# huster-wgm/SRCGAN

Hardware: AMD Instinct MI355X
Metric: paired SR-CycleGAN train images/sec at x4 256->1024 (higher is better)
Workload: dtype bf16; 1 GPU; Sat2Aerx4 paired G+D step (BASELINE configs[1]): 23-block RRDB generator + 3-layer PatchGAN, 3x256x256->3x1024x1024, batch 16/GPU; per_gpu_batch=16, global_batch=16, parallelism=dp1, gradient_exchange=none (1 rank)

## Files before the change

include/srcgan_amd.h:

```cpp
#ifndef SRCGAN_AMD_H
#define SRCGAN_AMD_H

#include <stddef.h>
#include <stdint.h>

#ifdef __cplusplus
extern "C" {
#endif

#define SRCGAN_F32 0
#define SRCGAN_BF16 1
#define SRCGAN_F16 2

int srcgan_version(void);
const char* srcgan_last_error(void);
int srcgan_dtype_size(int dtype);

int srcgan_nchw_f32_to_nhwc(const float* src, void* dst, int B, int C, int H, int W,
                            int cs, int dtype, void* stream);
int srcgan_nhwc_to_nchw_f32(const void* src, float* dst, int B, int C, int H, int W,
                            int cs, int coff, int dtype, void* stream);

size_t srcgan_packed_weight_bytes(int rows, int kdim, int ntaps, int dtype);
int srcgan_pack_weight(const float* w, void* wp, int rows, int kdim, int tys, int txs,
// ... 39 lines not shown
size_t srcgan_conv_wgrad_slab_bytes(int Cout, int Cin, int kh, int kw, int nsplit);
int srcgan_conv_wgrad_nsplit(int B, int OH, int OW, int Cout, int Cin, int stride);
int srcgan_conv_wgrad(const srcgan_wgrad_desc* d, void* stream);

typedef struct srcgan_wgrad_seg { int g0, g1; float* grad; float* bias; int Cin; float alpha; } srcgan_wgrad_seg;
typedef struct srcgan_wgrad_dense_desc {
    const void* dy; const void* x; float* slab;
    int dtype;
    int B, H, W;
    int G, dy_cs, dy_coff;
    int C, x_cs, x_coff;
    int nseg;
    srcgan_wgrad_seg seg[8];
    int accumulate;
    long dy_plane, x_plane;
} srcgan_wgrad_dense_desc;
size_t srcgan_wgrad_dense_slab_bytes(int G, int C, int dtype, int B, int H, int W);
int srcgan_wgrad_dense(const srcgan_wgrad_dense_desc* d, void* stream);

int srcgan_col_reduce_blocks(long npix);
int srcgan_col_reduce(int mode, const void* a, int a_cs, int a_coff, const void* z, int z_cs, int z_coff,
                      const float* m, const float* rstd, long npix, int C, float scale,
                      float* out0, float* out1, float* scratch, int dtype, void* stream);

int srcgan_bn_finalize(const float* mean, const float* var, float* rstd, float* running_mean,
                       float* running_var, int64_t* num_batches_tracked, int C, long count,
                       float momentum, float eps, void* stream);
int srcgan_bn_eval_rstd(const float* running_var, float* rstd, int C, float eps, void* stream);
int srcgan_bn_apply_lrelu(const void* z, void* y, const float* mean, const float* rstd, const float* gamma,
                          const float* beta, long npix, int C, int cs, float slope, int dtype, void* stream);
int srcgan_bn_bwd_apply(const void* g, const void* z, void* dz, const float* mean, const float* rstd,
                        const float* gamma, const float* sum_g, const float* sum_gx, long npix, int C, int cs,
                        int dtype, void* stream);

int srcgan_add_inplace(void* y, int y_cs, int y_coff, const void* x, int x_cs, int x_coff,
                       const void* mz, int mz_cs, int mz_coff, float mslope, long npix, int C, int dtype, void* stream);
int srcgan_add_inplace_planes(void* y, int y_cs, int y_coff, long y_plane, const void* x, int x_cs, int x_coff, long x_plane,
                              const void* mz, int mz_cs, int mz_coff, long mz_plane, float mslope, long npix, int C,
                              int dtype, void* stream);

size_t srcgan_gn_scratch_floats(int B, int C);
int srcgan_gn_forward(const void* x, int x_cs, const void* res, int res_cs, void* y, int y_cs, const float* gamma, const float* beta,
                      float* stats, int B, long hw, int C, int G, float eps, int relu, float slope, int dtype, float* scratch, void* stream);
int srcgan_gn_backward(const void* dy, int dy_cs, const void* yact, int ya_cs, const void* x, int x_cs, const float* gamma, const float* stats,
                       void* dx, int dx_cs, void* dres, int dres_cs, int dres_accumulate, float* dgamma, float* dbeta, int accumulate,
                       float slope, int B, long hw, int C, int G, int dtype, float* scratch, void* stream);

size_t srcgan_ca_scratch_floats(int B, long hw, int C);
int srcgan_ca_forward(const void* t, int t_cs, const void* res, int res_cs, void* y, int y_cs, const float* w1, const float* b1,
                      const float* w2, const float* b2, float* saved, int B, long hw, int C, int Cr, int dtype, float* scratch, void* stream);
int srcgan_ca_backward(const void* dy, int dy_cs, const void* t, int t_cs, const float* w1, const float* w2, const float* saved, void* dt,
                       int dt_cs, void* dres, int dres_cs, int dres_accumulate, float* dw1, float* db1, float* dw2, float* db2, int B,
                       long hw, int C, int Cr, int dtype, float* scratch, void* stream);

int srcgan_s2d_shift(const void* x, int x_cs, void* g, int g_cs, int B, int Hx, int Wx, int C, int s, int shift, int Hg, int Wg, int dtype, void* stream);
int srcgan_d2s_shift(const void* g, int g_cs, void* y, int y_cs, int B, int Hy, int Wy, int C, int s, int shift, int Hg, int Wg, int accumulate, int dtype,
                     void* stream);
int srcgan_prelu_forward(const void* z, int z_cs, const float* slope, const float* bias, const void* r, int r_cs, float beta, void* y, int y_cs, int B,
                         int Hy, int Wy, int C, int s, int shift, int Hg, int Wg, int dtype, void* stream);
size_t srcgan_prelu_scratch_floats(int B, int Hg, int Wg, int C, int s);
int srcgan_prelu_backward(const void* dy, int dy_cs, const void* z, int z_cs, const float* slope, const float* bias, void* dz, int dz_cs, void* dres,
                          int dres_cs, float beta, int dres_accumulate, float* dslope, float* dbias, int B, int Hy, int Wy, int C, int s, int shift,
                          int Hg, int Wg, int dtype, float* scratch, void* stream);

int srcgan_upsample2_nhwc(const void* src, int s_cs, int s_coff, long s_plane, void* dst, int d_cs,
                          int B, int H, int W, int C, int dtype, void* stream);
// ... 336 lines not shown
```

srcgan_amd/_native.py:

```python
from __future__ import annotations

import ctypes as C
import os
from typing import Optional, Sequence

import torch

_HERE = os.path.dirname(os.path.abspath(__file__))
LIB_PATH = os.environ.get("SRCGAN_AMD_LIB") or os.path.join(_HERE, "lib", "libsrcgan_amd.so")

F32, BF16, F16 = 0, 1, 2
_DTYPES = {"fp32": F32, "f32": F32, "float32": F32, torch.float32: F32,
           "bf16": BF16, "bfloat16": BF16, torch.bfloat16: BF16,
           "fp16": F16, "f16": F16, "float16": F16, "half": F16, torch.float16: F16, F32: F32, BF16: BF16, F16: F16}
_default_dtype = _DTYPES[os.environ.get("SRCGAN_AMD_DTYPE", "fp32")]


def dtype_id(d) -> int:
    if d is None:
        return _default_dtype
    try:
        return _DTYPES[d]
    except KeyError:
        raise ValueError(f"unsupported compute dtype {d!r} (use 'fp32', 'bf16' or 'fp16')") from None
# ... 95 lines not shown


class VggLossCfg(C.Structure):
    _fields_ = [(n, C.c_int) for n in ("kind", "B", "H", "W", "dtype")]


class NLayerDCfg(C.Structure):
    _fields_ = [("in_ch", C.c_int), ("ndf", C.c_int), ("n_layers", C.c_int),
                ("B", C.c_int), ("H", C.c_int), ("W", C.c_int), ("dtype", C.c_int), ("training", C.c_int), ("norm", C.c_int)]


_P, _I, _L, _F, _S = C.c_void_p, C.c_int, C.c_long, C.c_float, C.c_size_t
SIGNATURES = {
    "srcgan_version": (_I, []),
    "srcgan_last_error": (C.c_char_p, []),
    "srcgan_dtype_size": (_I, [_I]),
    "srcgan_nchw_f32_to_nhwc": (_I, [_P, _P, _I, _I, _I, _I, _I, _I, _P]),
    "srcgan_nhwc_to_nchw_f32": (_I, [_P, _P, _I, _I, _I, _I, _I, _I, _I, _P]),
    "srcgan_packed_weight_bytes": (_S, [_I, _I, _I, _I]),
    "srcgan_pack_weight": (_I, [_P, _P, _I, _I, _I, _I, _L, _L, _L, _L, _L, _I, _P]),
    "srcgan_pack_weight_part": (_I, [_P, _P, _I, _I, _I, _I, _L, _L, _L, _L, _L, _I, _I, _F, _I, _P]),
    "srcgan_conv_igemm": (_I, [C.POINTER(ConvDesc), _P]),
    "srcgan_conv_wgrad_slab_bytes": (_S, [_I, _I, _I, _I, _I]),
    "srcgan_conv_wgrad_nsplit": (_I, [_I, _I, _I, _I, _I, _I]),
    "srcgan_conv_wgrad": (_I, [C.POINTER(WgradDesc), _P]),
    "srcgan_wgrad_dense_slab_bytes": (_S, [_I, _I, _I, _I, _I, _I]),
    "srcgan_wgrad_dense": (_I, [C.POINTER(WgradDenseDesc), _P]),
    "srcgan_col_reduce_blocks": (_I, [_L]),
    "srcgan_col_reduce": (_I, [_I, _P, _I, _I, _P, _I, _I, _P, _P, _L, _I, _F, _P, _P, _P, _I, _P]),
    "srcgan_bn_finalize": (_I, [_P, _P, _P, _P, _P, _P, _I, _L, _F, _F, _P]),
    "srcgan_bn_eval_rstd": (_I, [_P, _P, _I, _F, _P]),
    "srcgan_bn_apply_lrelu": (_I, [_P, _P, _P, _P, _P, _P, _L, _I, _I, _F, _I, _P]),
    "srcgan_bn_bwd_apply": (_I, [_P, _P, _P, _P, _P, _P, _P, _P, _L, _I, _I, _I, _P]),
    "srcgan_add_inplace": (_I, [_P, _I, _I, _P, _I, _I, _P, _I, _I, _F, _L, _I, _I, _P]),
    "srcgan_add_inplace_planes": (_I, [_P, _I, _I, _L, _P, _I, _I, _L, _P, _I, _I, _L, _F, _L, _I, _I, _P]),
    "srcgan_gn_scratch_floats": (_S, [_I, _I]),
    "srcgan_gn_forward": (_I, [_P, _I, _P, _I, _P, _I, _P, _P, _P, _I, _L, _I, _I, _F, _I, _F, _I, _P, _P]),
    "srcgan_gn_backward": (_I, [_P, _I, _P, _I, _P, _I, _P, _P, _P, _I, _P, _I, _I, _P, _P, _I, _F, _I, _L, _I, _I, _I, _P, _P]),
    "srcgan_ca_scratch_floats": (_S, [_I, _L, _I]),
    "srcgan_ca_forward": (_I, [_P, _I, _P, _I, _P, _I, _P, _P, _P, _P, _P, _I, _L, _I, _I, _I, _P, _P]),
    "srcgan_ca_backward": (_I, [_P, _I, _P, _I, _P, _P, _P, _P, _I, _P, _I, _I, _P, _P, _P, _P, _I, _L, _I, _I, _I, _P, _P]),
    "srcgan_s2d_shift": (_I, [_P, _I, _P, _I, _I, _I, _I, _I, _I, _I, _I, _I, _I, _P]),
    "srcgan_d2s_shift": (_I, [_P, _I, _P, _I, _I, _I, _I, _I, _I, _I, _I, _I, _I, _I, _P]),
    "srcgan_prelu_forward": (_I, [_P, _I, _P, _P, _P, _I, _F, _P, _I, _I, _I, _I, _I, _I, _I, _I, _I, _I, _P]),
    "srcgan_prelu_scratch_floats": (_S, [_I, _I, _I, _I, _I]),
    "srcgan_prelu_backward": (_I, [_P, _I, _P, _I, _P, _P, _P, _I, _P, _I, _F, _I, _P, _P, _I, _I, _I, _I, _I, _I, _I, _I, _I, _P, _P]),
    "srcgan_reflect_pad_nhwc": (_I, [_P, _I, _P, _I, _I, _I, _I, _I, _I, _I, _P]),
    "srcgan_reflect_pad_bwd_nhwc": (_I, [_P, _I, _P, _I, _I, _I, _I, _I, _I, _I, _I, _P]),
    "srcgan_tanh_forward": (_I, [_P, _I, _P, _I, _L, _I, _I, _P]),
    "srcgan_tanh_backward": (_I, [_P, _I, _P, _I, _P, _I, _L, _I, _I, _I, _P]),
    "srcgan_upsample2_nhwc": (_I, [_P, _I, _I, _L, _P, _I, _I, _I, _I, _I, _I, _P]),
    "srcgan_sum2x2_nhwc": (_I, [_P, _I, _P, _I, _P, _I, _F, _I, _I, _I, _I, _I, _P]),
    "srcgan_loss_scratch_floats": (_I, []),
    "srcgan_loss_fwd": (_I, [_I, _P, _P, _F, _L, _P, _P, _P]),
    "srcgan_loss_bwd": (_I, [_I, _P, _P, _F, _L, _P, _F, _P, _P]),
    "srcgan_psnr_from_mse": (_I, [_P, _P, _P]),
    "srcgan_focal_fwd": (_I, [_P, _P, _L, _I, _F, _I, _P, _P, _P]),
    "srcgan_focal_bwd": (_I, [_P, _P, _L, _I, _F, _I, _P, _P, _P]),
    "srcgan_bce_fwd": (_I, [_P, _P, _L, _P, _P, _P]),
    "srcgan_bce_bwd": (_I, [_P, _P, _L, _P, _P, _P]),
    "srcgan_nll_argmax_fwd": (_I, [_P, _P, _I, _I, _L, _P, _P, _P]),
    "srcgan_nll_argmax_bwd": (_I, [_P, _P, _I, _I, _L, _P, _P, _P]),
    "srcgan_batch_range_fwd": (_I, [_P, _I, _L, _P, _P, _P]),
    "srcgan_batch_range_bwd": (_I, [_P, _I, _L, _P, _P, _P]),
    "srcgan_cross_l1_fwd": (_I, [_P, _P, _I, _L, _P, _P, _P]),
    "srcgan_cross_l1_bwd": (_I, [_P, _P, _I, _L, _P, _P, _P]),
# ... 85 lines not shown


for _stem, _cfg in (("resdeconv", ResDeconvCfg), ("srnet", SrNetCfg), ("srdense", SrDenseCfg), ("rcan", RcanCfg), ("ddbpn", DdbpnCfg), ("rdn", RdnCfg),
                    ("mdsr", MdsrCfg), ("vdsr", VdsrCfg), ("resnetgen", ResnetGenCfg)):
    SIGNATURES.update(_train_rows(_stem, _cfg))
for _stem, _cfg in (("srnet", SrNetCfg), ("rcan", RcanCfg), ("ddbpn", DdbpnCfg), ("rdn", RdnCfg),
                    ("mdsr", MdsrCfg), ("vdsr", VdsrCfg), ("resnetgen", ResnetGenCfg)):
    SIGNATURES.update(_infer_rows(_stem, _cfg))
SIGNATURES.update({
    "srcgan_resdeconv_infer_ws_bytes": (_S, [C.POINTER(ResDeconvCfg), _I]),
    "srcgan_resdeconv_infer_act_bytes": (_S, [C.POINTER(ResDeconvCfg), _I]),
    "srcgan_resdeconv_infer_plan": (_I, [C.POINTER(ResDeconvCfg), _I, C.POINTER(C.c_size_t), _I]),
    "srcgan_resdeconv_infer": (_I, [C.POINTER(ResDeconvCfg), _P, _P, _P, _P, _I, _P]),
    "srcgan_srdense_out_hw": (_I, [C.POINTER(SrDenseCfg), C.POINTER(C.c_int), C.POINTER(C.c_int)]),
    "srcgan_srdense_infer_ws_bytes": (_S, [C.POINTER(SrDenseCfg)]),
    "srcgan_srdense_infer": (_I, [C.POINTER(SrDenseCfg), _P, _P, _P, _P, _P]),
})

_lib = None


def lib() -> C.CDLL:
    global _lib
    if _lib is None:
        if not os.path.exists(LIB_PATH):
            raise RuntimeError(
                f"srcgan_amd: native library {LIB_PATH} is missing. Build it with "
                "`python -m srcgan_amd.build` (hipcc --offload-arch=gfx950). There is no CPU fallback.")
        handle = C.CDLL(LIB_PATH)
        for name, (res, args) in SIGNATURES.items():
            fn = getattr(handle, name)
            fn.restype, fn.argtypes = res, args
        _lib = handle
    return _lib


def check(rc: int, what: str) -> None:
    if rc != 0:
        msg = lib().srcgan_last_error()
        raise RuntimeError(f"srcgan_amd: {what} failed: {msg.decode() if msg else 'unknown error'}")


def stream_ptr(device=None) -> int:
    return torch.cuda.current_stream(device).cuda_stream


def require_cuda(t: torch.Tensor, what: str) -> None:
    if not t.is_cuda:
        raise RuntimeError(
            f"srcgan_amd: {what} got a {t.device} tensor. The native path runs on an MI355X GPU only; "
            "there is no CPU fallback (move the module and its inputs to 'cuda').")


def scene_layout(x):
    if not isinstance(x, torch.Tensor):
        return None
    if x.dtype == torch.uint8 and x.dim() in (2, 3):
        v = x if x.dim() == 3 else x[:, :, None]
        return "u8", v, int(v.shape[2]), int(v.shape[0]), int(v.shape[1])
    if x.dtype == torch.float32 and (x.dim() == 3 or (x.dim() == 4 and x.shape[0] == 1)):
        v = x if x.dim() == 3 else x[0]
        return "f32", v, int(v.shape[0]), int(v.shape[1]), int(v.shape[2])
    return None


def ptr_array(tensors: Sequence[Optional[torch.Tensor]]):
    arr = (C.c_void_p * len(tensors))()
    for i, t in enumerate(tensors):
        arr[i] = None if t is None else t.data_ptr()
    return arr


def workspace(nbytes: int, device) -> torch.Tensor:
    if nbytes <= 0:
        raise RuntimeError("srcgan_amd: native planner rejected the configuration: "
                           + (lib().srcgan_last_error() or b"").decode())
    return torch.empty(nbytes, dtype=torch.uint8, device=device)


def prof_enable(on: bool) -> None:
    check(lib().srcgan_prof_enable(int(on)), "srcgan_prof_enable")


def prof_collect():
    l = lib()
    out = []
    for i in range(l.srcgan_prof_collect()):
        cls, cnt, ms, fl, by = C.c_char_p(), C.c_long(), C.c_double(), C.c_double(), C.c_double()
        check(l.srcgan_prof_get(i, C.byref(cls), C.byref(cnt), C.byref(ms), C.byref(fl), C.byref(by)), "srcgan_prof_get")
        out.append({"cls": cls.value.decode(), "count": cnt.value, "ms": ms.value, "flops": fl.value, "bytes": by.value})
    return out
```

srcgan_amd/build.py:

```python
import glob
import os
import subprocess
import sys
from concurrent.futures import ThreadPoolExecutor

HERE = os.path.dirname(os.path.abspath(__file__))
CSRC = os.path.join(HERE, "csrc")
LIBDIR = os.path.join(HERE, "lib")
LIB = os.path.join(LIBDIR, "libsrcgan_amd.so")
SOURCES = ["conv_entry.hip", "conv_igemm.hip", "conv_par4.hip", "deconv_k3s2.hip", "conv3x3_dma.hip", "conv_wgrad.hip", "wgrad_dense.hip", "elementwise.hip", "class_losses.hip", "groupnorm.hip", "chan_attn.hip", "back_proj.hip", "reflect_pad.hip", "metrics.hip", "shift_select.hip", "scene_score.hip", "colour.hip", "tiles.hip", "vgg_loss.hip", "nets.hip", "oplist.hip"]
FLAGS = ["--offload-arch=gfx950", "-O3", "-std=c++17", "-fPIC", "-Wall", "-Wno-unused-function"]


def _hipcc():
    for c in (os.environ.get("HIPCC"), "/opt/rocm/bin/hipcc", "hipcc"):
        if c and (os.path.isabs(c) and os.path.exists(c) or not os.path.isabs(c)):
            return c
    raise RuntimeError("hipcc not found")


def _stale(target, deps):
    if not os.path.exists(target):
        return True
    t = os.path.getmtime(target)
    return any(os.path.getmtime(d) > t for d in deps)


def build(force=False, verbose=True):
    os.makedirs(LIBDIR, exist_ok=True)
    hipcc = _hipcc()
    headers = glob.glob(os.path.join(CSRC, "*.h")) + [os.path.join(HERE, "..", "include", "srcgan_amd.h")]
    objs, jobs = [], []
    for s in SOURCES:
        src = os.path.join(CSRC, s)
        obj = os.path.join(LIBDIR, s.replace(".hip", ".o"))
        objs.append(obj)
        if force or _stale(obj, [src] + headers):
            jobs.append([hipcc, *FLAGS, "-c", src, "-o", obj])

    def run(cmd):
        if verbose:
            print("[srcgan_amd.build]", " ".join(cmd), flush=True)
        subprocess.run(cmd, check=True)
# ... 13 lines not shown
```

srcgan_amd/csrc/common.h:

```cpp
#pragma once
#include <hip/hip_runtime.h>
#include <stdint.h>
#include <stdio.h>
#include <stdarg.h>
#include <string.h>
#include "../../include/srcgan_amd.h"

typedef __attribute__((ext_vector_type(8))) __bf16 bf16x8;
typedef __attribute__((ext_vector_type(8))) _Float16 f16x8;
typedef __attribute__((ext_vector_type(4))) _Float16 f16x4;
typedef __attribute__((ext_vector_type(4))) __bf16 bf16x4;
typedef __attribute__((ext_vector_type(4))) float f32x4;
typedef __attribute__((ext_vector_type(16))) float f32x16;
typedef __attribute__((ext_vector_type(4))) short s16x4;
typedef __attribute__((ext_vector_type(4))) unsigned int u32x4;
typedef __attribute__((ext_vector_type(2))) unsigned int u32x2;

template <typename T> struct DT;
template <> struct DT<float>  { static constexpr int id = SRCGAN_F32;  static constexpr int EPP = 4; static constexpr int KCE = 16; };
template <> struct DT<__bf16> { static constexpr int id = SRCGAN_BF16; static constexpr int EPP = 8; static constexpr int KCE = 32; };
template <> struct DT<_Float16> { static constexpr int id = SRCGAN_F16; static constexpr int EPP = 8; static constexpr int KCE = 32; };
static inline bool sg_is16(int dtype) { return dtype == SRCGAN_BF16 || dtype == SRCGAN_F16; }
static inline bool sg_dtype_ok(int dtype) { return dtype == SRCGAN_F32 || sg_is16(dtype); }

// ... 89 lines not shown
#ifdef SG_DIAG
#include <stdlib.h>
#define SG_DBG(p, bit) ((p).dbg & (bit))
static inline const char* sg_env(const char* name) { return getenv(name); }
#else
#define SG_DBG(p, bit) 0
static inline const char* sg_env(const char*) { return nullptr; }
#if defined(SG_TRACE) || defined(SG_WD_EXP) || defined(SG_EXP_NO_HALO_DMA) || defined(SG_EXP_NO_WEIGHT_DMA) || defined(SG_EXP_B_KX0_ONLY) || \
    defined(SG_EXP_NO_FRAG_READS) || defined(SG_EXP_NO_MFMA_INSTR)
#error "timing experiments need -DSG_DIAG (scripts/build_variant.sh adds it)"
#endif
#endif

int sg_prof_start(const char* cls, double flops, double bytes, hipStream_t st);
void sg_prof_stop(int token, hipStream_t st);

struct SgPackJob {
    const float* w; size_t wp_off;
    int rows, kdim, tys, txs;
    long sr, sk, sty, stx, off;
    int k_off, k_total; float scale;
    int cot, nchunk; long total, blk0;
};
void sg_pack_job_finish(SgPackJob& j, int dtype, long& blk_cursor);
int sg_pack_multi_launch(const SgPackJob* jobs_dev, int njobs, long nblocks, void* wp_base, int dtype, hipStream_t st, const unsigned long long* guard = nullptr);
int sg_fold_tail_pack(const float* w_deconv, const float* w_conv, void* wp, int tar, int dtype, hipStream_t st);
void sg_minmax_frames(const float* x, int planes, int frames, long n, int nblk, float* partial, float* range, hipStream_t st);
int sg_vgg_combine(const float* sums, const float* weights, int n, float* out, hipStream_t st);
struct SgFrames { int Cin, F, f0, k; };
int sg_frames_pack(const float* src5d, void* dst, int cs, int Bt, SgFrames fr, int H, int W, int dtype, hipStream_t st);
int sg_frames_grad_store(const void* src, int cs, float* dst5d, int Bt, SgFrames fr, int H, int W, const float* gout, float gscale, int dtype, hipStream_t st);
int sg_meanshift(const void* x, void* y, const float* w, const float* bias, int transpose, long npix, int dtype, hipStream_t st);
int sg_proj_repack(const float* src, float* dst, int form, int rows, int kdim, int k, int s, int back, hipStream_t st);
int sg_fill_zero_guarded(void* p, size_t bytes, const unsigned long long* guard, hipStream_t st);
```

srcgan_amd/csrc/elementwise.hip:

```cpp
#include "common.h"
#include "pixel_ops.h"

static thread_local char g_err[512] = "";
void srcgan_set_error(const char* fmt, ...) {
    va_list ap; va_start(ap, fmt); vsnprintf(g_err, sizeof(g_err), fmt, ap); va_end(ap);
}
extern "C" const char* srcgan_last_error(void) { return g_err; }
extern "C" int srcgan_version(void) { return 100; }
extern "C" int srcgan_dtype_size(int dtype) { return dtype == SRCGAN_F32 ? 4 : (sg_is16(dtype) ? 2 : 0); }

#include <vector>
#include <string>
#include <map>
namespace {
struct ProfRec { std::string cls; double flops, bytes; hipEvent_t e0, e1; };
bool g_prof_on = false;
std::vector<ProfRec> g_prof;
struct ProfAgg { std::string cls; long count; double ms, flops, bytes; };
std::vector<ProfAgg> g_agg;
}
int sg_prof_start(const char* cls, double flops, double bytes, hipStream_t st) {
    if (!g_prof_on) return -1;
    ProfRec r; r.cls = cls; r.flops = flops; r.bytes = bytes;
    if (hipEventCreate(&r.e0) != hipSuccess || hipEventCreate(&r.e1) != hipSuccess) return -1;
// ... 590 lines not shown
        partial[(size_t)blockIdx.x * C + c] = mean;
        partial[((size_t)gridDim.x + blockIdx.x) * C + c] = m2;
    }
}
__global__ __launch_bounds__(256) void col_meanvar_finalize_k(const float* __restrict__ partial, int nblk, int C, long npix,
                                                              float* __restrict__ mean_out, float* __restrict__ var_out) {
    __shared__ float red[3][32][8];
    const int cx = threadIdx.x & 7, py = threadIdx.x >> 3;
    const int c = blockIdx.x * 8 + cx;
    const long per = cdivl(npix, (long)nblk);
    auto count = [&](int b) { const long p0 = (long)b * per, p1 = (p0 + per < npix) ? p0 + per : npix; return p1 > p0 ? (float)(p1 - p0) : 0.f; };
    float n = 0.f, mean = 0.f, m2 = 0.f;
    if (c < C) {
        int b = py;
        for (; b + 96 < nblk; b += 128) {
            float mb[4], qb[4];
#pragma unroll
            for (int u = 0; u < 4; ++u) { mb[u] = partial[(size_t)(b + 32 * u) * C + c]; qb[u] = partial[((size_t)nblk + b + 32 * u) * C + c]; }
#pragma unroll
            for (int u = 0; u < 4; ++u) chan_combine(n, mean, m2, count(b + 32 * u), mb[u], qb[u]);
        }
        for (; b < nblk; b += 32) chan_combine(n, mean, m2, count(b), partial[(size_t)b * C + c], partial[((size_t)nblk + b) * C + c]);
    }
    red[0][py][cx] = n; red[1][py][cx] = mean; red[2][py][cx] = m2;
    __syncthreads();
    if (py == 0 && c < C) {
        float nn = 0.f, mm = 0.f, qq = 0.f;
        for (int q = 0; q < 32; ++q) chan_combine(nn, mm, qq, red[0][q][cx], red[1][q][cx], red[2][q][cx]);
        mean_out[c] = mm;
        var_out[c] = qq / (float)npix;
    }
}

extern "C" int srcgan_col_reduce_blocks(long npix) {
    long b = cdivl(npix, 256);
    return (int)(b > 512 ? 512 : (b < 1 ? 1 : b));
}

extern "C" int srcgan_col_reduce(int mode, const void* a, int a_cs, int a_coff, const void* z, int z_cs, int z_coff,
                                 const float* m, const float* rstd, long npix, int C, float scale,
                                 float* out0, float* out1, float* scratch, int dtype, void* stream) {
    SG_REQUIRE(a && out0 && scratch && npix > 0 && C > 0, "srcgan_col_reduce: bad arguments");
    SG_REQUIRE(mode >= 0 && mode <= 3, "srcgan_col_reduce: bad mode %d", mode);
    SG_REQUIRE(mode == 0 || mode == 3 || m, "srcgan_col_reduce: mode %d needs mean", mode);
    SG_REQUIRE(mode != 2 || (z && rstd && out1), "srcgan_col_reduce: mode 2 needs z, rstd, out1");
    SG_REQUIRE(mode != 3 || out1, "srcgan_col_reduce: mode 3 needs out1 (variance)");
    const int nblk = srcgan_col_reduce_blocks(npix);
    hipStream_t st = (hipStream_t)stream;
    const int epp = dtype == SRCGAN_F32 ? 4 : 8;
    const bool vec = C % epp == 0 && 256 % (C / epp) == 0 && a_cs % epp == 0 && a_coff % epp == 0 && ((uintptr_t)a % 16) == 0 &&
                     (mode != 2 || (z_cs % epp == 0 && z_coff % epp == 0 && ((uintptr_t)z % 16) == 0));
    if (mode == 3) {
        if (!vec) {
            SG_TRY(srcgan_col_reduce(0, a, a_cs, a_coff, nullptr, 0, 0, nullptr, nullptr, npix, C, 1.f / (float)npix, out0, nullptr, scratch, dtype, stream));
            return srcgan_col_reduce(1, a, a_cs, a_coff, nullptr, 0, 0, out0, nullptr, npix, C, 1.f / (float)npix, out1, nullptr, scratch, dtype, stream);
        }
        DISPATCH_DTYPE(dtype, hipLaunchKernelGGL(col_meanvar_vec_k<T>, dim3(nblk), dim3(256), 0, st, (const T*)a, a_cs, a_coff, npix, C, scratch));
        SG_LAUNCH_CHECK();
        hipLaunchKernelGGL(col_meanvar_finalize_k, dim3(cdiv(C, 8)), dim3(256), 0, st, scratch, nblk, C, npix, out0, out1);
        SG_LAUNCH_CHECK();
        return 0;
    }
    if (vec) {
        DISPATCH_DTYPE(dtype, {
            if (mode == 0) hipLaunchKernelGGL((col_reduce_vec_k<T, 0>), dim3(nblk), dim3(256), 0, st, (const T*)a, a_cs, a_coff, (const T*)z, z_cs, z_coff, m, rstd, npix, C, scratch);
            else if (mode == 1) hipLaunchKernelGGL((col_reduce_vec_k<T, 1>), dim3(nblk), dim3(256), 0, st, (const T*)a, a_cs, a_coff, (const T*)z, z_cs, z_coff, m, rstd, npix, C, scratch);
            else hipLaunchKernelGGL((col_reduce_vec_k<T, 2>), dim3(nblk), dim3(256), 0, st, (const T*)a, a_cs, a_coff, (const T*)z, z_cs, z_coff, m, rstd, npix, C, scratch);
        });
    } else
    DISPATCH_DTYPE(dtype, {
        if (mode == 0) hipLaunchKernelGGL((col_reduce_k<T, 0>), dim3(nblk), dim3(256), 0, st, (const T*)a, a_cs, a_coff, (const T*)z, z_cs, z_coff, m, rstd, npix, C, scratch);
        else if (mode == 1) hipLaunchKernelGGL((col_reduce_k<T, 1>), dim3(nblk), dim3(256), 0, st, (const T*)a, a_cs, a_coff, (const T*)z, z_cs, z_coff, m, rstd, npix, C, scratch);
        else hipLaunchKernelGGL((col_reduce_k<T, 2>), dim3(nblk), dim3(256), 0, st, (const T*)a, a_cs, a_coff, (const T*)z, z_cs, z_coff, m, rstd, npix, C, scratch);
    });
    SG_LAUNCH_CHECK();
    hipLaunchKernelGGL(col_finalize_k, dim3(cdiv(C, 8)), dim3(256), 0, st, scratch, nblk, C, scale, out0, mode == 2 ? out1 : nullptr);
    SG_LAUNCH_CHECK();
    return 0;
}

__global__ void bn_finalize_k(const float* mean, const float* var, float* rstd, float* rmean, float* rvar,
                              int64_t* nbt, int C, float unbias, float momentum, float eps) {
    const int c = blockIdx.x * 256 + threadIdx.x;
    if (c == 0 && nbt) *nbt += 1;
    if (c >= C) return;
    rstd[c] = rsqrtf(var[c] + eps);
    if (rmean) rmean[c] = (1.f - momentum) * rmean[c] + momentum * mean[c];
    if (rvar) rvar[c] = (1.f - momentum) * rvar[c] + momentum * var[c] * unbias;
}

extern "C" int srcgan_bn_finalize(const float* mean, const float* var, float* rstd, float* running_mean, float* running_var,
                                  int64_t* nbt, int C, long count, float momentum, float eps, void* stream) {
    SG_REQUIRE(mean && var && rstd && C > 0 && count > 0, "srcgan_bn_finalize: bad arguments");
    const float unbias = count > 1 ? (float)((double)count / (double)(count - 1)) : 1.f;
    hipLaunchKernelGGL(bn_finalize_k, dim3(cdiv(C, 256)), dim3(256), 0, (hipStream_t)stream, mean, var, rstd,
                       running_mean, running_var, nbt, C, unbias, momentum, eps);
    SG_LAUNCH_CHECK();
    return 0;
}

__global__ void bn_eval_rstd_k(const float* rvar, float* rstd, int C, float eps) {
    const int c = blockIdx.x * 256 + threadIdx.x;
    if (c < C) rstd[c] = rsqrtf(rvar[c] + eps);
}
extern "C" int srcgan_bn_eval_rstd(const float* running_var, float* rstd, int C, float eps, void* stream) {
    SG_REQUIRE(running_var && rstd && C > 0, "srcgan_bn_eval_rstd: bad arguments");
    hipLaunchKernelGGL(bn_eval_rstd_k, dim3(cdiv(C, 256)), dim3(256), 0, (hipStream_t)stream, running_var, rstd, C, eps);
    SG_LAUNCH_CHECK();
    return 0;
}

// ... 528 lines not shown
```

srcgan_amd/csrc/nets.hip:

```cpp
#include "net_common.h"
#include <map>
#include <mutex>
#include <string>

int sg_zigzag_next() {
    static const bool zig = sg_env("SRCGAN_NO_ZIGZAG") == nullptr;
    static int flip = 0;
    const int rev = flip;
    flip ^= 1;
    return zig ? rev : 0;
}

namespace {
struct PackCache { std::vector<SgPackJob> host; SgPackJob* dev = nullptr; SgPackJob* pinned = nullptr; size_t cap = 0; hipEvent_t staged = nullptr; };
std::map<std::string, PackCache> g_pack_cache;
std::mutex g_pack_mutex;
}

int sg_pack_list_run(const std::vector<SgPackJob>& jobs, long nblk, void* wp_base, int dtype, const char* tag, const void* key_ptr, void* st,
                     const unsigned long long* guard) {
    if (jobs.empty()) return 0;
    int dev = 0;
    SG_HIP(hipGetDevice(&dev));
    char key[112];
// ... 843 lines not shown
        return srcgan_nhwc_to_nchw_f32(w8 + yl.Y, y_nchw, B, 1, yl.OH, yl.OW, yl.out_cs, 0, dt, st);
    }
    int pack_dgrad(bool pack_dx) const {
        PackList packs(dt, wp);
        for (int l = pack_dx ? 0 : 1; l < P.L; ++l) {
            const DLayer& y = P.y[l];
            if (y.folded) {
                const int cin = c->in_ch, cout = y.Cout, kce = 64 / P.esz;
                SG_TRY(sg_fill_zero_guarded(wp + y.wd[0], y.wd_bytes, pack_guard(opt), (hipStream_t)st));
                for (int q = 0; q < 4; ++q)
                    for (int hk = 0; hk < 2; ++hk)
                        packs.add(params[y.pw], wp + y.wd[0] + (size_t)q * 8 * kce * P.esz, cin, cout / 2, 2, 2, 16, (long)cin * 16, -8, -2,
                                  10 + (q >> 1) * 4 + (q & 1) + (long)hk * (cout / 2) * cin * 16, hk * (cout / 2), cout);
            } else if (y.stride == 1)
                packs.add(params[y.pw], wp + y.wd[0], y.Cin, y.Cout, y.k, y.k, lay_dgrad_s1(y.Cin, y.k, y.k));
            else
                y.s2().pack(packs, params[y.pw], wp, y.wd);
        }
        return packs.run(P.s2d() ? (pack_dx ? "d_bwd_dx_s2d" : "d_bwd_s2d") : (pack_dx ? "d_bwd_dx" : "d_bwd"), params[0], st, pack_guard(opt));
    }
    int norm_backward(const DLayer& y, TRef dcur) const {
        const int C = y.Cout;
        const long npix = (long)B * y.OH * y.OW;
        if (y.post == D_INORM)
            return srcgan_gn_backward(dcur.p, dcur.cs, nullptr, 0, w8 + y.Z, C, nullptr, W(y.stat), dcur.p, dcur.cs, nullptr, 0, 0,
                                      nullptr, nullptr, 0, 0.2f, B, (long)y.OH * y.OW, C, C, dt, S(Q->gnscr), st);
        if (y.post != D_BNORM) return 0;
        float* mean = W(y.stat); float* rstd = mean + 2 * C; float* sums = S(Q->sums);
        SG_TRY(srcgan_col_reduce(2, dcur.p, dcur.cs, 0, w8 + y.Z, C, 0, mean, rstd, npix, C, 1.f, sums, sums + C, S(Q->colscr), dt, st));
        if (grads[y.pbeta]) SG_HIP(hipMemcpyAsync(grads[y.pbeta], sums, C * sizeof(float), hipMemcpyDeviceToDevice, (hipStream_t)st));
        if (grads[y.pg]) SG_HIP(hipMemcpyAsync(grads[y.pg], sums + C, C * sizeof(float), hipMemcpyDeviceToDevice, (hipStream_t)st));
        return srcgan_bn_bwd_apply(dcur.p, w8 + y.Z, dcur.p, mean, rstd, params[y.pg], sums, sums + C, npix, C, C, dt, st);
    }
    int param_grads(const DLayer& y, TRef dcur) const {
        if (grads[y.pw]) {
            float* g = y.folded ? S(Q->gfold) : grads[y.pw];
            SG_TRY(wgrad_call(dt, dcur, y.OH, y.OW, y.Cout, X(y), B, y.H, y.W, y.Cin, y.k, y.k, y.stride, y.pad, y.pad, lay_fwd(y.Cin, y.k, y.k), 1.f, S(Q->slab), g, st));
            if (y.folded) SG_TRY(srcgan_s2d_wgrad_unfold(g, grads[y.pw], y.Cout, c->in_ch, 0, st));
        }
        if (y.pb >= 0 && grads[y.pb]) SG_TRY(bias_grad(dt, dcur, (long)B * y.OH * y.OW, y.Cout, 1.f, grads[y.pb], S(Q->colscr), st));
        return 0;
    }
    int input_grad(const DLayer& y, TRef dcur, TRef dst, TRef mz) const {
        if (y.stride == 2) return y.s2().run(dt, dcur, B, y.OH, y.OW, dst, y.H, y.W, wp, y.wd, TNULL, mz, true, st);
        Conv cv(dt, y.k, y.k, 1);
        cv.in(dcur, B, y.OH, y.OW, y.out_cs).w(wp + y.wd[0]).out(dst, y.H, y.W, y.Cin).pad(y.k - 1 - y.pad, y.k - 1 - y.pad);
        if (mz.p) cv.mask(mz, 0);
        return cv.run(st);
    }
    int write_dx(TRef dcur, float* dx_nchw) const {
        const DLayer& y = P.y[0];
        TRef dxin = tref(s8 + Q->dxin, y.in_cs);
        if (!P.s2d())
            SG_HIP(hipMemsetAsync(dxin.p, 0, (size_t)B * y.H * y.W * y.in_cs * P.esz, (hipStream_t)st));
        SG_TRY(input_grad(y, dcur, dxin, TNULL));
        if (P.s2d()) return srcgan_s2d_to_nchw_f32(dxin.p, dx_nchw, B, c->in_ch, c->H, c->W, dt, st);
        return srcgan_nhwc_to_nchw_f32(dxin.p, dx_nchw, B, c->in_ch, c->H, c->W, y.in_cs, 0, dt, st);
    }
    int backward(const float* dy_nchw, float* dx_nchw) const {
        if (do_pack) SG_TRY(pack_dgrad(dx_nchw || (opt && opt->wpack)));
        const DLayer& yl = P.y[P.L - 1];
        TRef dcur = tref(s8 + Q->dO, yl.out_cs);
        SG_TRY(srcgan_nchw_f32_to_nhwc(dy_nchw, dcur.p, B, 1, yl.OH, yl.OW, yl.out_cs, dt, st));
        for (int l = P.L - 1; l > 0; --l) {
            const DLayer& y = P.y[l];
            TRef dst = tref(s8 + Q->g[l & 1], y.Cin);
            SG_TRY(norm_backward(y, dcur));
            SG_TRY(param_grads(y, dcur));
            SG_TRY(input_grad(y, dcur, dst, X(y)));
            dcur = dst;
        }
        SG_TRY(param_grads(P.y[0], dcur));
        if (dx_nchw) SG_TRY(write_dx(dcur, dx_nchw));
        return 0;
    }
};
}

extern "C" int srcgan_nlayerd_num_params(const srcgan_nlayerd_cfg* c) { DPlan P; if (d_plan(c, P)) return -1; return P.nparams; }
extern "C" int srcgan_nlayerd_out_hw(const srcgan_nlayerd_cfg* c, int* oh, int* ow) {
    DPlan P; SG_TRY(d_plan(c, P)); if (oh) *oh = P.y[P.L - 1].OH; if (ow) *ow = P.y[P.L - 1].OW; return 0;
}
extern "C" size_t srcgan_nlayerd_ws_bytes(const srcgan_nlayerd_cfg* c) { DPlan P; if (d_plan(c, P)) return 0; return P.total; }
extern "C" size_t srcgan_nlayerd_bwd_scratch_bytes(const srcgan_nlayerd_cfg* c) {
    DPlan P; if (d_plan(c, P)) return 0; DBwdPlan Q; d_bwd_plan(c, P, Q); return Q.total;
}
extern "C" size_t srcgan_nlayerd_wpack_bytes(const srcgan_nlayerd_cfg* c) { DPlan P; if (d_plan(c, P)) return 0; return P.total - P.wpk; }

extern "C" int srcgan_nlayerd_forward(const srcgan_nlayerd_cfg* c, const float* x_nchw, const float* const* params,
                                      float* const* bn_running, int64_t* const* bn_nbt, void* ws, float* y_nchw, void* st) {
    return srcgan_nlayerd_forward_ex(c, x_nchw, params, bn_running, bn_nbt, ws, y_nchw, nullptr, st);
}
extern "C" int srcgan_nlayerd_backward(const srcgan_nlayerd_cfg* c, const float* dy_nchw, const float* const* params,
                                       void* ws, void* scratch, float* const* grads, float* dx_nchw, void* st) {
    return srcgan_nlayerd_backward_ex(c, dy_nchw, params, ws, scratch, grads, dx_nchw, nullptr, st);
}

extern "C" int srcgan_nlayerd_forward_ex(const srcgan_nlayerd_cfg* c, const float* x_nchw, const float* const* params,
                                         float* const* bn_running, int64_t* const* bn_nbt, void* ws, float* y_nchw,
                                         const srcgan_net_opts* opt, void* st) {
    DPlan P;
    SG_TRY(d_plan(c, P));
// ... 18 lines not shown
```

Baseline: 119.6 images/s.

## Fuse PatchGAN final 1-channel conv dgrad into BN+LeakyReLU backward

Adds a pred_head kernel pair that recomputes the final 4x4, 1-output-channel conv's input gradient on the fly from the tiny dy map and the weights. This path is fused with the preceding BatchNorm/LeakyReLU backward (column sums, then apply), so the dgrad conv launch, the dcur activation-gradient tensor and its round trip through memory are no longer needed. The gradient is recomputed in both the sums and apply passes, trading some redundant FMAs for lower memory traffic. An env switch can restore the old route.

Result: no change. 120.1 images/s (median of 6 runs) (+0.4%).

```diff
diff --git a/include/srcgan_amd.h b/include/srcgan_amd.h
--- a/include/srcgan_amd.h
+++ b/include/srcgan_amd.h
@@ -95,6 +95,15 @@
 int srcgan_bn_bwd_apply(const void* g, const void* z, void* dz, const float* mean, const float* rstd,
                         const float* gamma, const float* sum_g, const float* sum_gx, long npix, int C, int cs,
                         int dtype, void* stream);
+
+int srcgan_set_narrow_route(int old_route);
+int srcgan_bn_bwd_head_ok(int C, int dtype);
+int srcgan_bn_bwd_head_sums(const float* dy, const float* w, const void* z, const void* y_act, const float* mean, const float* rstd,
+                            const float* gamma, const float* beta, int B, int H, int W, int C, float slope,
+                            float* sum_g, float* sum_gx, float* scratch, int dtype, void* stream);
+int srcgan_bn_bwd_head_apply(const float* dy, const float* w, const void* z, const void* y_act, void* dz, const float* mean,
+                             const float* rstd, const float* gamma, const float* beta, const float* sum_g, const float* sum_gx,
+                             int B, int H, int W, int C, float slope, int dtype, void* stream);
 
 int srcgan_add_inplace(void* y, int y_cs, int y_coff, const void* x, int x_cs, int x_coff,
                        const void* mz, int mz_cs, int mz_coff, float mslope, long npix, int C, int dtype, void* stream);
diff --git a/srcgan_amd/_native.py b/srcgan_amd/_native.py
--- a/srcgan_amd/_native.py
+++ b/srcgan_amd/_native.py
@@ -151,6 +151,10 @@
     "srcgan_bn_eval_rstd": (_I, [_P, _P, _I, _F, _P]),
     "srcgan_bn_apply_lrelu": (_I, [_P, _P, _P, _P, _P, _P, _L, _I, _I, _F, _I, _P]),
     "srcgan_bn_bwd_apply": (_I, [_P, _P, _P, _P, _P, _P, _P, _P, _L, _I, _I, _I, _P]),
+    "srcgan_set_narrow_route": (_I, [_I]),
+    "srcgan_bn_bwd_head_ok": (_I, [_I, _I]),
+    "srcgan_bn_bwd_head_sums": (_I, [_P, _P, _P, _P, _P, _P, _P, _P, _I, _I, _I, _I, _F, _P, _P, _P, _I, _P]),
+    "srcgan_bn_bwd_head_apply": (_I, [_P, _P, _P, _P, _P, _P, _P, _P, _P, _P, _P, _I, _I, _I, _I, _F, _I, _P]),
     "srcgan_add_inplace": (_I, [_P, _I, _I, _P, _I, _I, _P, _I, _I, _F, _L, _I, _I, _P]),
     "srcgan_add_inplace_planes": (_I, [_P, _I, _I, _L, _P, _I, _I, _L, _P, _I, _I, _L, _F, _L, _I, _I, _P]),
     "srcgan_gn_scratch_floats": (_S, [_I, _I]),
@@ -302,6 +306,8 @@
             fn = getattr(handle, name)
             fn.restype, fn.argtypes = res, args
         _lib = handle
+        if os.environ.get("SRCGAN_AMD_NARROW_ROUTE") == "old":
+            handle.srcgan_set_narrow_route(1)
     return _lib
 
 
@@ -348,6 +354,10 @@
     return torch.empty(nbytes, dtype=torch.uint8, device=device)
 
 
+def set_narrow_route(old_route: bool) -> bool:
+    return bool(lib().srcgan_set_narrow_route(int(bool(old_route))))
+
+
 def prof_enable(on: bool) -> None:
     check(lib().srcgan_prof_enable(int(on)), "srcgan_prof_enable")
 
diff --git a/srcgan_amd/build.py b/srcgan_amd/build.py
--- a/srcgan_amd/build.py
+++ b/srcgan_amd/build.py
@@ -8,7 +8,7 @@
 CSRC = os.path.join(HERE, "csrc")
 LIBDIR = os.path.join(HERE, "lib")
 LIB = os.path.join(LIBDIR, "libsrcgan_amd.so")
-SOURCES = ["conv_entry.hip", "conv_igemm.hip", "conv_par4.hip", "deconv_k3s2.hip", "conv3x3_dma.hip", "conv_wgrad.hip", "wgrad_dense.hip", "elementwise.hip", "class_losses.hip", "groupnorm.hip", "chan_attn.hip", "back_proj.hip", "reflect_pad.hip", "metrics.hip", "shift_select.hip", "scene_score.hip", "colour.hip", "tiles.hip", "vgg_loss.hip", "nets.hip", "oplist.hip"]
+SOURCES = ["conv_entry.hip", "conv_igemm.hip", "conv_par4.hip", "deconv_k3s2.hip", "conv3x3_dma.hip", "conv_wgrad.hip", "wgrad_dense.hip", "elementwise.hip", "pred_head.hip", "class_losses.hip", "groupnorm.hip", "chan_attn.hip", "back_proj.hip", "reflect_pad.hip", "metrics.hip", "shift_select.hip", "scene_score.hip", "colour.hip", "tiles.hip", "vgg_loss.hip", "nets.hip", "oplist.hip"]
 FLAGS = ["--offload-arch=gfx950", "-O3", "-std=c++17", "-fPIC", "-Wall", "-Wno-unused-function"]
 
 
diff --git a/srcgan_amd/csrc/common.h b/srcgan_amd/csrc/common.h
--- a/srcgan_amd/csrc/common.h
+++ b/srcgan_amd/csrc/common.h
@@ -145,4 +145,6 @@
 int sg_frames_grad_store(const void* src, int cs, float* dst5d, int Bt, SgFrames fr, int H, int W, const float* gout, float gscale, int dtype, hipStream_t st);
 int sg_meanshift(const void* x, void* y, const float* w, const float* bias, int transpose, long npix, int dtype, hipStream_t st);
 int sg_proj_repack(const float* src, float* dst, int form, int rows, int kdim, int k, int s, int back, hipStream_t st);
+int sg_col_finalize(const float* partial, int nblk, int C, float scale, float* out0, float* out1, hipStream_t st);
+bool sg_narrow_old_route();
 int sg_fill_zero_guarded(void* p, size_t bytes, const unsigned long long* guard, hipStream_t st);
diff --git a/srcgan_amd/csrc/elementwise.hip b/srcgan_amd/csrc/elementwise.hip
--- a/srcgan_amd/csrc/elementwise.hip
+++ b/srcgan_amd/csrc/elementwise.hip
@@ -646,6 +646,12 @@
     }
 }
 
+int sg_col_finalize(const float* partial, int nblk, int C, float scale, float* out0, float* out1, hipStream_t st) {
+    hipLaunchKernelGGL(col_finalize_k, dim3(cdiv(C, 8)), dim3(256), 0, st, partial, nblk, C, scale, out0, out1);
+    SG_LAUNCH_CHECK();
+    return 0;
+}
+
 extern "C" int srcgan_col_reduce_blocks(long npix) {
     long b = cdivl(npix, 256);
     return (int)(b > 512 ? 512 : (b < 1 ? 1 : b));
@@ -688,9 +694,7 @@
         else hipLaunchKernelGGL((col_reduce_k<T, 2>), dim3(nblk), dim3(256), 0, st, (const T*)a, a_cs, a_coff, (const T*)z, z_cs, z_coff, m, rstd, npix, C, scratch);
     });
     SG_LAUNCH_CHECK();
-    hipLaunchKernelGGL(col_finalize_k, dim3(cdiv(C, 8)), dim3(256), 0, st, scratch, nblk, C, scale, out0, mode == 2 ? out1 : nullptr);
-    SG_LAUNCH_CHECK();
-    return 0;
+    return sg_col_finalize(scratch, nblk, C, scale, out0, mode == 2 ? out1 : nullptr, st);
 }
 
 __global__ void bn_finalize_k(const float* mean, const float* var, float* rstd, float* rmean, float* rvar,
diff --git a/srcgan_amd/csrc/nets.hip b/srcgan_amd/csrc/nets.hip
--- a/srcgan_amd/csrc/nets.hip
+++ b/srcgan_amd/csrc/nets.hip
@@ -899,6 +899,22 @@
         if (grads[y.pg]) SG_HIP(hipMemcpyAsync(grads[y.pg], sums + C, C * sizeof(float), hipMemcpyDeviceToDevice, (hipStream_t)st));
         return srcgan_bn_bwd_apply(dcur.p, w8 + y.Z, dcur.p, mean, rstd, params[y.pg], sums, sums + C, npix, C, C, dt, st);
     }
+    bool head_fused() const {
+        const DLayer& yl = P.y[P.L - 1]; const DLayer& yb = P.y[P.L - 2];
+        return !sg_narrow_old_route() && yl.post == D_FINAL && yl.Cout == 1 && yl.k == 4 && yl.stride == 1 && yl.pad == 1 &&
+               yb.post == D_BNORM && c->training && srcgan_bn_bwd_head_ok(yb.Cout, dt);
+    }
+    int head_norm_backward(const DLayer& yb, const float* dy_nchw, TRef dst) const {
+        const DLayer& yl = P.y[P.L - 1];
+        const int C = yb.Cout;
+        float* mean = W(yb.stat); float* rstd = mean + 2 * C; float* sums = S(Q->sums);
+        SG_TRY(srcgan_bn_bwd_head_sums(dy_nchw, params[yl.pw], w8 + yb.Z, nullptr, mean, rstd, params[yb.pg], params[yb.pbeta], B, yb.OH, yb.OW, C,
+                                       0.2f, sums, sums + C, S(Q->colscr), dt, st));
+        if (grads[yb.pbeta]) SG_HIP(hipMemcpyAsync(grads[yb.pbeta], sums, C * sizeof(float), hipMemcpyDeviceToDevice, (hipStream_t)st));
+        if (grads[yb.pg]) SG_HIP(hipMemcpyAsync(grads[yb.pg], sums + C, C * sizeof(float), hipMemcpyDeviceToDevice, (hipStream_t)st));
+        return srcgan_bn_bwd_head_apply(dy_nchw, params[yl.pw], w8 + yb.Z, nullptr, dst.p, mean, rstd, params[yb.pg], params[yb.pbeta], sums, sums + C,
+                                        B, yb.OH, yb.OW, C, 0.2f, dt, st);
+    }
     int param_grads(const DLayer& y, TRef dcur) const {
         if (grads[y.pw]) {
             float* g = y.folded ? S(Q->gfold) : grads[y.pw];
@@ -929,12 +945,14 @@
         const DLayer& yl = P.y[P.L - 1];
         TRef dcur = tref(s8 + Q->dO, yl.out_cs);
         SG_TRY(srcgan_nchw_f32_to_nhwc(dy_nchw, dcur.p, B, 1, yl.OH, yl.OW, yl.out_cs, dt, st));
+        const bool fused = head_fused();
         for (int l = P.L - 1; l > 0; --l) {
             const DLayer& y = P.y[l];
             TRef dst = tref(s8 + Q->g[l & 1], y.Cin);
-            SG_TRY(norm_backward(y, dcur));
+            if (!(fused && l == P.L - 2)) SG_TRY(norm_backward(y, dcur));
             SG_TRY(param_grads(y, dcur));
-            SG_TRY(input_grad(y, dcur, dst, X(y)));
+            if (fused && l == P.L - 1) SG_TRY(head_norm_backward(P.y[l - 1], dy_nchw, dst));
+            else SG_TRY(input_grad(y, dcur, dst, X(y)));
             dcur = dst;
         }
         SG_TRY(param_grads(P.y[0], dcur));
diff --git a/srcgan_amd/csrc/pred_head.hip b/srcgan_amd/csrc/pred_head.hip
--- /dev/null
+++ b/srcgan_amd/csrc/pred_head.hip
@@ -0,0 +1,243 @@
+#include "common.h"
+
+namespace {
+constexpr int HB_CH = 256;
+
+int g_narrow_old = 0;
+
+__device__ __forceinline__ void head_stage(f32x4 (*pat)[4], const float* __restrict__ dy, long q0, int n, int H, int W) {
+    const int j = threadIdx.x;
+    if (j >= n) return;
+    const long q = q0 + j, r = q / W;
+    const int x = (int)(q - r * W), y = (int)(r % H), OH = H - 1, OW = W - 1;
+    const float* d = dy + (r / H) * ((long)OH * OW);
+#pragma unroll
+    for (int ky = 0; ky < 4; ++ky) {
+        const int oy = y + 1 - ky;
+        f32x4 v;
+#pragma unroll
+        for (int kx = 0; kx < 4; ++kx) {
+            const int ox = x + 1 - kx;
+            v[kx] = (oy >= 0 && oy < OH && ox >= 0 && ox < OW) ? d[(long)oy * OW + ox] : 0.f;
+        }
+        pat[j][ky] = v;
+    }
+}
+
+__device__ __forceinline__ float head_dot(const float (&w)[16], const f32x4 (&p)[4]) {
+    float a = 0.f;
+#pragma unroll
+    for (int t = 0; t < 16; ++t) a = __builtin_fmaf(w[t], p[t >> 2][t & 3], a);
+    return a;
+}
+
+template <typename T> struct HeadChan {
+    static constexpr int EPP = DT<T>::EPP;
+    float w[EPP][16], sc[EPP], sh[EPP], mu[EPP];
+    __device__ __forceinline__ void load(const float* __restrict__ wt, const float* __restrict__ mean, const float* __restrict__ rstd,
+                                         const float* __restrict__ gamma, const float* __restrict__ beta, int c0) {
+#pragma unroll
+        for (int i = 0; i < EPP; ++i) {
+#pragma unroll
+            for (int t = 0; t < 16; ++t) w[i][t] = wt[(c0 + i) * 16 + t];
+            sc[i] = rstd[c0 + i] * gamma[c0 + i];
+            sh[i] = __builtin_fmaf(-mean[c0 + i], sc[i], beta[c0 + i]);
+            mu[i] = mean[c0 + i];
+        }
+    }
+    template <bool FROM_Y> __device__ __forceinline__ float g(int i, const f32x4 (&p)[4], float zf, float yf, float slope) const {
+        bool pos;
+        if (FROM_Y) pos = yf > 0.f;
+        else { const float u = __builtin_fmaf(zf, sc[i], sh[i]); pos = u > 0.f && to_f(from_f<T>(u)) > 0.f; }
+        return head_dot(w[i], p) * (pos ? 1.f : slope);
+    }
+};
+
+template <typename T, bool FROM_Y>
+__global__ __launch_bounds__(256, 2) void bn_bwd_head_sums_k(const float* __restrict__ dy, const float* __restrict__ wt, const T* __restrict__ z,
+                                                          const T* __restrict__ yact, const float* __restrict__ mean,
+                                                          const float* __restrict__ rstd, const float* __restrict__ gamma,
+                                                          const float* __restrict__ beta, int H, int W, int C, long npix, float slope,
+                                                          float* __restrict__ partial) {
+    constexpr int EPP = DT<T>::EPP, UN = EPP == 8 ? 2 : 4;
+    typedef __attribute__((ext_vector_type(EPP))) T vecT;
+    __shared__ f32x4 pat[HB_CH][4];
+    __shared__ float red[2][256 * EPP];
+    const int G = C / EPP, PL = 256 / G;
+    const int cg = threadIdx.x % G, pl = threadIdx.x / G, c0 = cg * EPP;
+    const long per = cdivl(npix, gridDim.x);
+    const long p0 = (long)blockIdx.x * per, p1 = (p0 + per < npix) ? p0 + per : npix;
+    HeadChan<T> k;
+    k.load(wt, mean, rstd, gamma, beta, c0);
+    float s0[EPP], s1[EPP];
+    typedef __attribute__((ext_vector_type(EPP))) float vecF;
+    volatile vecF* mus = (volatile vecF*)&red[0][threadIdx.x * EPP];
+    {
+        vecF m;
+#pragma unroll
+        for (int i = 0; i < EPP; ++i) { s0[i] = 0.f; s1[i] = 0.f; m[i] = k.mu[i]; }
+        *mus = m;
+    }
+    auto acc1 = [&](int j, const vecT& zv, const vecT& yv) {
+        const f32x4 p[4] = {pat[j][0], pat[j][1], pat[j][2], pat[j][3]};
+        const vecF mu = *mus;
+#pragma unroll
+        for (int i = 0; i < EPP; ++i) {
+            const float zf = to_f(zv[i]);
+            const float gv = k.template g<FROM_Y>(i, p, zf, to_f(yv[i]), slope);
+            s0[i] += gv; s1[i] += gv * (zf - mu[i]);
+        }
+    };
+    for (long q0 = p0; q0 < p1; q0 += HB_CH) {
+        const int n = (int)(p1 - q0 < HB_CH ? p1 - q0 : HB_CH);
+        __syncthreads();
+        head_stage(pat, dy, q0, n, H, W);
+        __syncthreads();
+        int j = pl;
+        for (; j + (UN - 1) * PL < n; j += UN * PL) {
+            vecT zv[UN], yv[UN];
+#pragma unroll
+            for (int u = 0; u < UN; ++u) {
+                zv[u] = *(const vecT*)(z + (size_t)(q0 + j + u * PL) * C + c0);
+                yv[u] = FROM_Y ? *(const vecT*)(yact + (size_t)(q0 + j + u * PL) * C + c0) : zv[u];
+            }
+#pragma unroll
+            for (int u = 0; u < UN; ++u) acc1(j + u * PL, zv[u], yv[u]);
+        }
+        for (; j < n; j += PL) {
+            const vecT zv = *(const vecT*)(z + (size_t)(q0 + j) * C + c0);
+            const vecT yv = FROM_Y ? *(const vecT*)(yact + (size_t)(q0 + j) * C + c0) : zv;
+            acc1(j, zv, yv);
+        }
+    }
+#pragma unroll
+    for (int i = 0; i < EPP; ++i) { red[0][threadIdx.x * EPP + i] = s0[i]; red[1][threadIdx.x * EPP + i] = s1[i] * rstd[c0 + i]; }
+    __syncthreads();
+    for (int c = threadIdx.x; c < C; c += 256) {
+        float t0 = 0.f, t1 = 0.f;
+        for (int q = 0; q < PL; ++q) { t0 += red[0][(q * G + c / EPP) * EPP + c % EPP]; t1 += red[1][(q * G + c / EPP) * EPP + c % EPP]; }
+        partial[(size_t)blockIdx.x * C + c] = t0;
+        partial[((size_t)gridDim.x + blockIdx.x) * C + c] = t1;
+    }
+}
+
+template <typename T, bool FROM_Y>
+__global__ __launch_bounds__(256, 2) void bn_bwd_head_apply_k(const float* __restrict__ dy, const float* __restrict__ wt, const T* __restrict__ z,
+                                                           const T* __restrict__ yact, T* __restrict__ dz, const float* __restrict__ mean,
+                                                           const float* __restrict__ rstd, const float* __restrict__ gamma,
+                                                           const float* __restrict__ beta, const float* __restrict__ sum_g,
+                                                           const float* __restrict__ sum_gx, int H, int W, int C, long npix, float invn,
+                                                           float slope) {
+    constexpr int EPP = DT<T>::EPP;
+    typedef __attribute__((ext_vector_type(EPP))) T vecT;
+    __shared__ f32x4 pat[HB_CH][4];
+    const int G = C / EPP, PL = 256 / G;
+    const int cg = threadIdx.x % G, pl = threadIdx.x / G, c0 = cg * EPP;
+    HeadChan<T> k;
+    k.load(wt, mean, rstd, gamma, beta, c0);
+    float ka[EPP], kb[EPP], kc[EPP];
+#pragma unroll
+    for (int i = 0; i < EPP; ++i) {
+        ka[i] = gamma[c0 + i] * rstd[c0 + i]; kb[i] = sum_g[c0 + i] * invn;
+        kc[i] = rstd[c0 + i] * sum_gx[c0 + i] * invn;
+    }
+    auto one = [&](long q0, int j, const vecT& zv, const vecT& yv) {
+        const f32x4 p[4] = {pat[j][0], pat[j][1], pat[j][2], pat[j][3]};
+        vecT o;
+#pragma unroll
+        for (int i = 0; i < EPP; ++i) {
+            const float zf = to_f(zv[i]);
+            const float gv = k.template g<FROM_Y>(i, p, zf, to_f(yv[i]), slope);
+            o[i] = from_f<T>(ka[i] * (gv - kb[i] - (zf - k.mu[i]) * kc[i]));
+        }
+        *(vecT*)(dz + (size_t)(q0 + j) * C + c0) = o;
+    };
+    for (long q0 = (long)blockIdx.x * HB_CH; q0 < npix; q0 += (long)gridDim.x * HB_CH) {
+        const int n = (int)(npix - q0 < HB_CH ? npix - q0 : HB_CH);
+        __syncthreads();
+        head_stage(pat, dy, q0, n, H, W);
+        __syncthreads();
+        int j = pl;
+        for (; j + 3 * PL < n; j += 4 * PL) {
+            vecT zv[4], yv[4];
+#pragma unroll
+            for (int u = 0; u < 4; ++u) {
+                zv[u] = *(const vecT*)(z + (size_t)(q0 + j + u * PL) * C + c0);
+                yv[u] = FROM_Y ? *(const vecT*)(yact + (size_t)(q0 + j + u * PL) * C + c0) : zv[u];
+            }
+#pragma unroll
+            for (int u = 0; u < 4; ++u) one(q0, j + u * PL, zv[u], yv[u]);
+        }
+        for (; j < n; j += PL) {
+            const vecT zv = *(const vecT*)(z + (size_t)(q0 + j) * C + c0);
+            const vecT yv = FROM_Y ? *(const vecT*)(yact + (size_t)(q0 + j) * C + c0) : zv;
+            one(q0, j, zv, yv);
+        }
+    }
+}
+
+template <typename T> const char* head_cls(const char* f32, const char* bf16, const char* f16) {
+    return sizeof(T) == 4 ? f32 : __is_same(T, __bf16) ? bf16 : f16;
+}
+}
+
+extern "C" int srcgan_set_narrow_route(int old_route) { const int was = g_narrow_old; g_narrow_old = old_route != 0; return was; }
+bool sg_narrow_old_route() { return g_narrow_old != 0; }
+
+extern "C" int srcgan_bn_bwd_head_ok(int C, int dtype) {
+    if (!sg_dtype_ok(dtype) || C <= 0) return 0;
+    const int epp = dtype == SRCGAN_F32 ? 4 : 8;
+    return C % epp == 0 && 256 % (C / epp) == 0;
+}
+
+#define HEAD_DISPATCH(dtype, ...) \
+    if ((dtype) == SRCGAN_F32) { using T = float; __VA_ARGS__; } \
+    else if ((dtype) == SRCGAN_BF16) { using T = __bf16; __VA_ARGS__; } \
+    else { using T = _Float16; __VA_ARGS__; }
+
+static int head_args_ok(const char* who, const void* dy, const void* w, const void* z, const void* y_act, int B, int H, int W, int C, int dtype) {
+    SG_REQUIRE(sg_dtype_ok(dtype), "%s: bad dtype %d", who, dtype);
+    SG_REQUIRE(dy && w && z && B > 0 && H >= 2 && W >= 2, "%s: bad arguments (the head's input must be at least 2x2)", who);
+    SG_REQUIRE(srcgan_bn_bwd_head_ok(C, dtype), "%s: needs C a multiple of one 16-byte vector, with C/vector dividing 256 (C=%d)", who, C);
+    SG_REQUIRE(((uintptr_t)z % 16) == 0 && ((uintptr_t)y_act % 16) == 0, "%s: z and y must be 16-byte aligned", who);
+    return 0;
+}
+
+extern "C" int srcgan_bn_bwd_head_sums(const float* dy, const float* w, const void* z, const void* y_act, const float* mean, const float* rstd,
+                                       const float* gamma, const float* beta, int B, int H, int W, int C, float slope,
+                                       float* sum_g, float* sum_gx, float* scratch, int dtype, void* stream) {
+    SG_TRY(head_args_ok("srcgan_bn_bwd_head_sums", dy, w, z, y_act, B, H, W, C, dtype));
+    SG_REQUIRE(mean && rstd && gamma && beta && sum_g && sum_gx && scratch, "srcgan_bn_bwd_head_sums: null pointer");
+    const long npix = (long)B * H * W;
+    const int nblk = srcgan_col_reduce_blocks(npix);
+    hipStream_t st = (hipStream_t)stream;
+    HEAD_DISPATCH(dtype, {
+        const int tok = sg_prof_start(head_cls<T>("bn_bwd_head_sums<f32>", "bn_bwd_head_sums<bf16>", "bn_bwd_head_sums<f16>"),
+                                      2.0 * 16 * npix * C, (double)npix * C * sizeof(T) * (y_act ? 2 : 1), st);
+        if (y_act) hipLaunchKernelGGL((bn_bwd_head_sums_k<T, true>), dim3(nblk), dim3(256), 0, st, dy, w, (const T*)z, (const T*)y_act, mean, rstd, gamma, beta, H, W, C, npix, slope, scratch);
+        else hipLaunchKernelGGL((bn_bwd_head_sums_k<T, false>), dim3(nblk), dim3(256), 0, st, dy, w, (const T*)z, (const T*)nullptr, mean, rstd, gamma, beta, H, W, C, npix, slope, scratch);
+        sg_prof_stop(tok, st);
+    });
+    SG_LAUNCH_CHECK();
+    return sg_col_finalize(scratch, nblk, C, 1.f, sum_g, sum_gx, st);
+}
+
+extern "C" int srcgan_bn_bwd_head_apply(const float* dy, const float* w, const void* z, const void* y_act, void* dz, const float* mean,
+                                        const float* rstd, const float* gamma, const float* beta, const float* sum_g, const float* sum_gx,
+                                        int B, int H, int W, int C, float slope, int dtype, void* stream) {
+    SG_TRY(head_args_ok("srcgan_bn_bwd_head_apply", dy, w, z, y_act, B, H, W, C, dtype));
+    SG_REQUIRE(dz && dz != z && ((uintptr_t)dz % 16) == 0 && mean && rstd && gamma && beta && sum_g && sum_gx, "srcgan_bn_bwd_head_apply: bad arguments");
+    const long npix = (long)B * H * W;
+    const long nch = cdivl(npix, HB_CH);
+    const int grid = (int)(nch < 2048 ? nch : 2048);
+    hipStream_t st = (hipStream_t)stream;
+    HEAD_DISPATCH(dtype, {
+        const int tok = sg_prof_start(head_cls<T>("bn_bwd_head_apply<f32>", "bn_bwd_head_apply<bf16>", "bn_bwd_head_apply<f16>"),
+                                      2.0 * 16 * npix * C, (double)npix * C * sizeof(T) * (y_act ? 3 : 2), st);
+        if (y_act) hipLaunchKernelGGL((bn_bwd_head_apply_k<T, true>), dim3(grid), dim3(256), 0, st, dy, w, (const T*)z, (const T*)y_act, (T*)dz, mean, rstd, gamma, beta, sum_g, sum_gx, H, W, C, npix, 1.f / (float)npix, slope);
+        else hipLaunchKernelGGL((bn_bwd_head_apply_k<T, false>), dim3(grid), dim3(256), 0, st, dy, w, (const T*)z, (const T*)nullptr, (T*)dz, mean, rstd, gamma, beta, sum_g, sum_gx, H, W, C, npix, 1.f / (float)npix, slope);
+        sg_prof_stop(tok, st);
+    });
+    SG_LAUNCH_CHECK();
+    return 0;
+}
```
